# OmerMersin/video-stab

Measured on AMD Instinct MI355X. Metric: stabilized frames/sec @1080p (whole job; warp-stage HBM GB/s in roofline), higher is better.
Workload: dtype u8

## Files before the change

video-stab_amd/csrc/k_lk.hip:

```cpp
#include "vs_common.h"

namespace vsd {
namespace {

constexpr int MAX_LEVELS = 8;

struct LKArgs {
    LKLevel levels[MAX_LEVELS];
    int max_level;
    const float* prev_pts;
    float* next_pts;
    uint8_t* status;
    float* err;
    int n;
    const int32_t* d_n;
    int win;
    int max_count;
    double eps2;
};

template <int CTRL>
__device__ __forceinline__ int dpp_mov(int v) {
    return __builtin_amdgcn_update_dpp(0, v, CTRL, 0xF, 0xF, true);
}
// ... 29 lines not shown
}

__device__ __forceinline__ int descale(int x, int n) { return (x + (1 << (n - 1))) >> n; }

struct Weights { int w00, w01, w10, w11; };

__device__ __forceinline__ Weights make_weights(float a, float b) {
    Weights w;
    w.w00 = f_round((1.f - a) * (1.f - b) * 16384.f);
    w.w01 = f_round(a * (1.f - b) * 16384.f);
    w.w10 = f_round((1.f - a) * b * 16384.f);
    w.w11 = 16384 - w.w00 - w.w01 - w.w10;
    return w;
}

__device__ __forceinline__ short2 load_deriv(const int16_t* __restrict__ d, int w, int h, int x, int y) {
    if ((unsigned)x >= (unsigned)w || (unsigned)y >= (unsigned)h) return make_short2(0, 0);
    return *reinterpret_cast<const short2*>(d + ((size_t)y * w + x) * 2);
}

typedef const __attribute__((address_space(1))) uint8_t* gmem_u8;
typedef const __attribute__((address_space(1))) int16_t* gmem_i16;
__device__ __forceinline__ gmem_u8 uniform_global(const uint8_t* p) {
    const unsigned long long v = (unsigned long long)p;
    const unsigned lo = (unsigned)__builtin_amdgcn_readfirstlane((int)(unsigned)v), hi = (unsigned)__builtin_amdgcn_readfirstlane((int)(unsigned)(v >> 32));
    return (gmem_u8)(((unsigned long long)hi << 32) | lo);
}

constexpr int LK_MARGIN = 6;
constexpr int LK_WIN_MAX = 31;



__device__ __forceinline__ void divmod_small(int i, int d, float inv_d, int& q, int& r) {
    q = (int)(((float)i + 0.5f) * inv_d);
    r = i - q * d;
}

template <int NPX>
__device__ __forceinline__ void lk_track(const LKArgs& a, const int pt) {
    constexpr int WM = NPX <= 4 ? 16 : (NPX <= 7 ? 21 : LK_WIN_MAX);
    constexpr int PWM = WM + 1, RWM = WM + 1 + 2 * LK_MARGIN;
    constexpr int PN = (PWM * PWM + 63) / 64, RN = (RWM * RWM + 63) / 64;
    __shared__ uint8_t pI[PN * 64];
    __shared__ short2 pD[PN * 64];
    __shared__ uint8_t region[RN * 64];
    const int lane = threadIdx.x;
    int n = a.n;
    if (a.d_n) { int dn = *a.d_n; n = dn < n ? dn : n; }
    if (pt >= n) return;
    const int win = a.win, area = win * win;
    const int PW = win + 1;
    const int RW = win + 1 + 2 * LK_MARGIN;
    const float inv_pw = 1.0f / (float)PW, inv_rw = 1.0f / (float)RW, inv_win = 1.0f / (float)win;
    uint32_t off[NPX];
#pragma unroll
    for (int k = 0; k < NPX; k++) {
        const int p = lane + 64 * k;
        int yy = 0, xx = 0;
        if (p < area) divmod_small(p, win, inv_win, yy, xx);
        off[k] = (uint32_t)(yy * PW + xx) | ((uint32_t)(yy * RW + xx) << 16);
    }
#define LK_VALID(k) (lane + 64 * (k) < area)
#define LK_POFF(k) ((int)(off[k] & 0xFFFFu))
#define LK_ROFF(k) ((int)(off[k] >> 16))
    int p_y0, p_x0, p_sy, p_sx, r_y0, r_x0, r_sy, r_sx;
    divmod_small(lane, PW, inv_pw, p_y0, p_x0);
    divmod_small(64, PW, inv_pw, p_sy, p_sx);
    divmod_small(lane, RW, inv_rw, r_y0, r_x0);
    divmod_small(64, RW, inv_rw, r_sy, r_sx);
    const float halfWin = (win - 1) * 0.5f;
    const float FLT_SCALE = 1.f / (1 << 20);
    const float px0 = a.prev_pts[2 * pt], py0 = a.prev_pts[2 * pt + 1];
    float outx = 0.f, outy = 0.f;
    int status = 1;
    float err = 0.f;

    for (int level = a.max_level; level >= 0; level--) {
        const LKLevel L = a.levels[level];
        const float scale = (float)(1. / (double)(1 << level));
        float prevx = px0 * scale, prevy = py0 * scale;
        if (level == a.max_level) { outx = prevx; outy = prevy; }
        else { outx = outx * 2.f; outy = outy * 2.f; }
        prevx -= halfWin; prevy -= halfWin;
        const int ipx = f_floor(prevx), ipy = f_floor(prevy);
        if (ipx < -win || ipx >= L.w || ipy < -win || ipy >= L.h) {
            if (level == 0) { status = 0; err = 0.f; }
            continue;
        }
        float cx = outx - halfWin, cy = outy - halfWin;
        int rx0 = f_floor(cx) - LK_MARGIN, ry0 = f_floor(cy) - LK_MARGIN;
        __syncthreads();
        const bool p_inside = ipx >= 0 && ipy >= 0 && ipx + PW <= L.w && ipy + PW <= L.h;
        if (p_inside) {
            const gmem_u8 pbase = uniform_global(L.prev + ((size_t)ipy * L.stride + ipx));
            const gmem_i16 dbase = (gmem_i16)uniform_global(reinterpret_cast<const uint8_t*>(L.deriv + ((size_t)ipy * L.w + ipx) * 2));
            constexpr int PB_ = 5;
            int y = p_y0, x = p_x0;
#pragma unroll
            for (int k0 = 0; k0 < PN; k0 += PB_) {
                uint8_t vI[PB_];
                uint32_t vD[PB_];
#pragma unroll
                for (int k = k0; k < k0 + PB_ && k < PN; k++) {
                    const bool ok = lane + 64 * k < PW * PW;
                    const uint32_t eo = ok ? (uint32_t)(y * (int)L.stride + x) : 0u, dof = ok ? (uint32_t)((y * L.w + x) * 2) : 0u;
                    vI[k - k0] = pbase[eo];
                    vD[k - k0] = *reinterpret_cast<const __attribute__((address_space(1))) uint32_t*>(dbase + dof);
                    x += p_sx; y += p_sy;
                    if (x >= PW) { x -= PW; y++; }
                }
#pragma unroll
                for (int k = k0; k < k0 + PB_ && k < PN; k++) { pI[lane + 64 * k] = vI[k - k0]; *reinterpret_cast<uint32_t*>(&pD[lane + 64 * k]) = vD[k - k0]; }
                __builtin_amdgcn_sched_barrier(0);
            }
        } else {
            int y = p_y0, x = p_x0;
            for (int i = lane; i < PW * PW; i += 64) {
                const int X = ipx + x, Y = ipy + y;
                pI[i] = L.prev[(size_t)reflect101(Y, L.h) * L.stride + reflect101(X, L.w)];
                pD[i] = load_deriv(L.deriv, L.w, L.h, X, Y);
                x += p_sx; y += p_sy;
                if (x >= PW) { x -= PW; y++; }
            }
        }
        auto stage_region = [&]() {
            const bool inside = rx0 >= 0 && ry0 >= 0 && rx0 + RW <= L.w && ry0 + RW <= L.h;
            int y = r_y0, x = r_x0;
            asm volatile("" : "+v"(x), "+v"(y));
            if (inside) {
                const gmem_u8 rbase = uniform_global(L.next + ((size_t)ry0 * L.stride + rx0));
                constexpr int RB_ = 10;
#pragma unroll
                for (int k0 = 0; k0 < RN; k0 += RB_) {
                    uint8_t vR[RB_];
#pragma unroll
                    for (int k = k0; k < k0 + RB_ && k < RN; k++) {
                        const bool ok = lane + 64 * k < RW * RW;
// ... 4 lines not shown
#pragma unroll
                    for (int k = k0; k < k0 + RB_ && k < RN; k++) region[lane + 64 * k] = vR[k - k0];
                    __builtin_amdgcn_sched_barrier(0);
                }
            } else {
                for (int i = lane; i < RW * RW; i += 64) {
                    const int X = rx0 + x, Y = ry0 + y;
                    region[i] = L.next[(size_t)reflect101(Y, L.h) * L.stride + reflect101(X, L.w)];
                    x += r_sx; y += r_sy;
                    if (x >= RW) { x -= RW; y++; }
                }
            }
        };
        stage_region();
        __syncthreads();
        Weights wt = make_weights(prevx - ipx, prevy - ipy);
        short Iw[NPX], Ix[NPX], Iy[NPX];
        int pA11 = 0, pA12 = 0, pA22 = 0;
#pragma unroll
        for (int k = 0; k < NPX; k++) {
            const int o = LK_POFF(k);
            int ival = descale(__mul24((int)pI[o], wt.w00) + __mul24((int)pI[o + 1], wt.w01) +
                               __mul24((int)pI[o + PW], wt.w10) + __mul24((int)pI[o + PW + 1], wt.w11), 9);
            const short2 d00 = pD[o], d01 = pD[o + 1], d10 = pD[o + PW], d11 = pD[o + PW + 1];
            int ixval = descale(__mul24((int)d00.x, wt.w00) + __mul24((int)d01.x, wt.w01) +
                                __mul24((int)d10.x, wt.w10) + __mul24((int)d11.x, wt.w11), 14);
            int iyval = descale(__mul24((int)d00.y, wt.w00) + __mul24((int)d01.y, wt.w01) +
                                __mul24((int)d10.y, wt.w10) + __mul24((int)d11.y, wt.w11), 14);
            if (!LK_VALID(k)) { ival = 0; ixval = 0; iyval = 0; }
            Iw[k] = (short)ival; Ix[k] = (short)ixval; Iy[k] = (short)iyval;
            pA11 += __mul24(ixval, ixval);
            pA12 += __mul24(ixval, iyval);
            pA22 += __mul24(iyval, iyval);
        }
        const long long sA11 = wave_sum(pA11), sA12 = wave_sum(pA12), sA22 = wave_sum(pA22);
        const float A11 = (float)sA11 * FLT_SCALE, A12 = (float)sA12 * FLT_SCALE, A22 = (float)sA22 * FLT_SCALE;
        float D = A11 * A22 - A12 * A12;
        const float minEig = (A22 + A11 - sqrtf((A11 - A22) * (A11 - A22) + 4.f * A12 * A12)) /
                             (float)(2 * win * win);
// ... 161 lines not shown
    if (!d_prev || !d_next || w <= 0 || h <= 0 || max_level < 0 || max_level >= MAX_LEVELS) {
        set_last_error("pyr_lk: invalid argument");
        return VS_ERR_INVALID_ARG;
    }
    int lw[MAX_LEVELS], lh[MAX_LEVELS];
    int levels = 0;
    {
        int sw = w, sh = h;
        for (int level = 0; level <= max_level; level++) {
            lw[level] = sw; lh[level] = sh;
            levels = level;
            sw = (sw + 1) / 2; sh = (sh + 1) / 2;
            if (sw <= win || sh <= win) break;
        }
    }
    size_t img_bytes = 0, der_bytes = 0;
    for (int i = 1; i <= levels; i++) img_bytes += (size_t)lw[i] * lh[i];
    for (int i = 0; i <= levels; i++) der_bytes += (size_t)lw[i] * lh[i] * 4;
    uint8_t* scratch = nullptr;
    const size_t total = 2 * img_bytes + der_bytes + 64;
    VS_HIP_TRY(hipMalloc((void**)&scratch, total));
    LKLevel L[MAX_LEVELS];
    uint8_t* pp = scratch;
    uint8_t* pn = scratch + img_bytes;
    int16_t* pd = reinterpret_cast<int16_t*>(scratch + ((2 * img_bytes + 15) & ~(size_t)15));
    int rc = VS_OK;
    for (int i = 0; i <= levels && rc == VS_OK; i++) {
        L[i].w = lw[i]; L[i].h = lh[i];
        if (i == 0) { L[i].prev = d_prev; L[i].next = d_next; L[i].stride = stride; }
        else {
            rc = launch_pyr_down(L[i - 1].prev, L[i - 1].stride, lw[i - 1], lh[i - 1], pp, lw[i], st);
            if (rc == VS_OK) rc = launch_pyr_down(L[i - 1].next, L[i - 1].stride, lw[i - 1], lh[i - 1], pn, lw[i], st);
            L[i].prev = pp; L[i].next = pn; L[i].stride = lw[i];
            pp += (size_t)lw[i] * lh[i]; pn += (size_t)lw[i] * lh[i];
        }
        if (rc == VS_OK) rc = launch_scharr(L[i].prev, L[i].stride, lw[i], lh[i], pd, st);
        L[i].deriv = pd;
        pd += (size_t)lw[i] * lh[i] * 2;
    }
    if (rc == VS_OK) rc = launch_pyr_lk(L, levels, d_prev_pts, n, nullptr, d_next_pts, d_status, d_err, win, max_iters, eps, st);
    hipError_t e = hipStreamSynchronize(st);
    (void)hipFree(scratch);
    if (rc == VS_OK && e != hipSuccess) { set_last_error(hipGetErrorString(e)); rc = VS_ERR_HIP; }
    return rc;
}

}
```

video-stab_amd/csrc/k_pyr.hip:

```cpp
#include "vs_common.h"

namespace vsd {
namespace {

constexpr int NT = 256;
constexpr int RPB = 4;

__global__ __launch_bounds__(NT) void pyr_down_kernel(const uint8_t* __restrict__ src_, size_t sstride,
                                                      int sw, int sh, uint8_t* __restrict__ dst_,
                                                      size_t dstride, int dw, int dh) {
    const uint8_t* __restrict__ src = src_;
    uint8_t* __restrict__ dst = dst_;
    const int x = blockIdx.x * blockDim.x + threadIdx.x;
    if (x >= dw) return;
    int xi[5];
#pragma unroll
    for (int k = 0; k < 5; k++) xi[k] = reflect101(2 * x + k - 2, sw);
    for (int y = blockIdx.y * RPB; y < min((int)(blockIdx.y + 1) * RPB, dh); y++) {
        int col[5];
#pragma unroll
        for (int j = 0; j < 5; j++) {
            const uint8_t* s = src + (size_t)reflect101(2 * y + j - 2, sh) * sstride;
            col[j] = s[xi[2]] * 6 + (s[xi[1]] + s[xi[3]]) * 4 + s[xi[0]] + s[xi[4]];
        }
// ... 17 lines not shown
    const int a_p = (r0[xp] + r2[xp]) * 3 + r1[xp] * 10;
    const int b_m = r2[xm] - r0[xm];
    const int b_c = r2[x] - r0[x];
    const int b_p = r2[xp] - r0[xp];
    short2 o;
    o.x = (short)(a_p - a_m);
    o.y = (short)((b_p + b_m) * 3 + b_c * 10);
    *reinterpret_cast<short2*>(dst + ((size_t)y * w + x) * 2) = o;
    }
}

constexpr int FT_W = 64, FT_H = 16;
constexpr int FT_PITCH = 72;
constexpr int FT_ROWS = FT_H + 4;

template <bool DOWN>
__global__ __launch_bounds__(NT) void pyr_level_kernel(const ImgPair* __restrict__ sch, const ImgPair* __restrict__ pyr, size_t sstride,
                                                       int w, int h, size_t dstride, int dw, int dh) {
    __shared__ __attribute__((aligned(16))) uint8_t tile[FT_ROWS * FT_PITCH];
    const uint8_t* __restrict__ src = static_cast<const uint8_t*>(sch[blockIdx.z].src);
    int16_t* __restrict__ der = static_cast<int16_t*>(sch[blockIdx.z].dst);
    const int tid = threadIdx.x;
    const int x0 = blockIdx.x * FT_W, y0 = blockIdx.y * FT_H;
    const bool inside = x0 >= 4 && y0 >= 2 && x0 + FT_W + 4 <= w && y0 + FT_H + 2 <= h && (sstride & 3) == 0 && ((uintptr_t)src & 3) == 0;
    if (inside) {
        constexpr int ND = (FT_ROWS * (FT_PITCH / 4) + NT - 1) / NT;
        uint32_t v[ND];
#pragma unroll
        for (int k = 0; k < ND; k++) {
            const int i = min(tid + NT * k, FT_ROWS * (FT_PITCH / 4) - 1);
            const int r = i / (FT_PITCH / 4), c4 = i - r * (FT_PITCH / 4);
            v[k] = *reinterpret_cast<const uint32_t*>(src + (size_t)(y0 - 2 + r) * sstride + (x0 - 4) + 4 * c4);
        }
#pragma unroll
        for (int k = 0; k < ND; k++)
            if (tid + NT * k < FT_ROWS * (FT_PITCH / 4)) reinterpret_cast<uint32_t*>(tile)[tid + NT * k] = v[k];
// ... 1 lines not shown
        constexpr int NB = (FT_ROWS + 2) / 3;
        const int c = tid % FT_PITCH, r0 = tid / FT_PITCH;
        const uint8_t* col = src + reflect101(x0 - 4 + c, w);
        size_t off[NB];
#pragma unroll
        for (int k = 0; k < NB; k++) off[k] = (size_t)reflect101(y0 - 2 + min(r0 + 3 * k, FT_ROWS - 1), h) * sstride;
        uint8_t v[NB];
#pragma unroll
        for (int k = 0; k < NB; k++) v[k] = col[off[k]];
#pragma unroll
        for (int k = 0; k < NB; k++)
            if (r0 + 3 * k < FT_ROWS) tile[(r0 + 3 * k) * FT_PITCH + c] = v[k];
    }
    __syncthreads();
    const uint32_t* T = reinterpret_cast<const uint32_t*>(tile);
    {
        const int r = tid >> 4, c = (tid & 15) * 4;
        const int y = y0 + r, x = x0 + c;
        if (y < h && x < w) {
            int t[3][6];
#pragma unroll
            for (int j = 0; j < 3; j++) {
                const uint32_t* q = T + (r + 1 + j) * (FT_PITCH / 4) + (c >> 2);
                const uint32_t lo = q[0], mid = q[1], hi = q[2];
                t[j][0] = lo >> 24;
                t[j][1] = mid & 255u; t[j][2] = (mid >> 8) & 255u; t[j][3] = (mid >> 16) & 255u; t[j][4] = mid >> 24;
                t[j][5] = hi & 255u;
            }
            int a[6], b[6];
#pragma unroll
            for (int k = 0; k < 6; k++) {
// ... 25 lines not shown
            for (int j = 0; j < 5; j++) {
                const uint32_t lo = q[j * (FT_PITCH / 4)], hi = q[j * (FT_PITCH / 4) + 1];
                const uint32_t four = __builtin_amdgcn_alignbyte(hi, lo, sh);
                const uint32_t fifth = (hi >> (8 * sh)) & 255u;
                col[j] = (int)__builtin_amdgcn_udot4(four, 0x04060401u, fifth, false);
            }
            dst[(size_t)yo * dstride + xo] = (uint8_t)((col[2] * 6 + (col[1] + col[3]) * 4 + col[0] + col[4] + 128) >> 8);
        }
    }
}

}

int launch_pyr_level_batch(const ImgPair* d_scharr_pairs, const ImgPair* d_pyr_pairs, int items, size_t sstride, int w, int h,
                           size_t dstride, hipStream_t st) {
    if (!d_scharr_pairs || items < 1 || items > 65535 || w <= 0 || h <= 0 || h > 65535) {
        set_last_error("pyr_level_batch: invalid argument");
        return VS_ERR_INVALID_ARG;
    }
    const int dw = (w + 1) / 2, dh = (h + 1) / 2;
    dim3 grid((w + FT_W - 1) / FT_W, (h + FT_H - 1) / FT_H, items);
    if (d_pyr_pairs) hipLaunchKernelGGL(pyr_level_kernel<true>, grid, dim3(NT), 0, st, d_scharr_pairs, d_pyr_pairs, sstride, w, h, dstride, dw, dh);
    else hipLaunchKernelGGL(pyr_level_kernel<false>, grid, dim3(NT), 0, st, d_scharr_pairs, d_pyr_pairs, sstride, w, h, dstride, dw, dh);
    VS_HIP_TRY(hipGetLastError());
    return VS_OK;
}

int launch_pyr_down(const uint8_t* d_src, size_t sstride, int sw, int sh, uint8_t* d_dst,
                    size_t dstride, hipStream_t st) {
    if (!d_src || !d_dst || sw <= 0 || sh <= 0 || sh > 131070) {
        set_last_error("pyr_down: invalid argument");
        return VS_ERR_INVALID_ARG;
    }
    const int dw = (sw + 1) / 2, dh = (sh + 1) / 2;
    dim3 grid((dw + NT - 1) / NT, (dh + RPB - 1) / RPB);
    hipLaunchKernelGGL(pyr_down_kernel, grid, dim3(NT), 0, st, d_src, sstride, sw, sh, d_dst, dstride, dw, dh);
    VS_HIP_TRY(hipGetLastError());
    return VS_OK;
// ... 15 lines not shown
```

video-stab_amd/csrc/stabilizer.cpp:

```cpp
#include <algorithm>
#include <array>
#include <atomic>
#include <cstring>
#include <cstdlib>
#include <deque>
#include <map>
#include <memory>
#include <mutex>
#include <new>
#include <vector>

#include "canvas.h"
#include "host_helper.h"
#include "traj_state.h"
#include "vs_common.h"
#include "warp_tab.h"

namespace vsd {

struct RansacTables;
int get_ransac_tables(int max_m, int iters, const RansacTables** out);
int launch_ransac(const float* d_from, const float* d_to, const uint8_t* d_status, int n, const int32_t* d_n,
                  float* d_vp, float* d_vc, int32_t* d_m, int min_points, double thr, int iters,
                  const RansacTables* tab, int32_t* d_counts, double* d_model, uint8_t* d_inliers,
// ... 32 lines not shown
int launch_fade_update(uint8_t* d_hist, const uint8_t* d_stab, size_t sstride, int row_bytes, int rows, hipStream_t st);
int launch_make_border(const uint8_t* src, size_t sstride, int w, int h, int cn, uint8_t* dst, size_t dstride,
                       int b, int border, hipStream_t st);
int launch_resize_linear(const uint8_t* d_src, size_t sstride, int sw, int sh, int cn, uint8_t* d_dst,
                         size_t dstride, int dw, int dh, hipStream_t st);

constexpr int FRAME_RING = 128;
constexpr int FRAME_RING_MAX = 192;
constexpr int MAX_PYR = 8;
constexpr int NPYR = 3;
constexpr int BATCH_MAX = 64;
constexpr int EVR = 4;

struct Pyramid {
    uint8_t* img[MAX_PYR] = {};
    int16_t* der[MAX_PYR] = {};
};

}

using namespace vsd;

struct vs_batch;
int group_drain(vs_batch* g);
int group_run(vs_batch* g);
bool group_holds_warps(const vs_batch* g);
vs_batch* group_new_own(vs_stab* s);
void group_delete(vs_batch* g);

struct vs_stab {
    vs_params_c p;
// ... 263 lines not shown
    s->items.assign(B, vs_stab::ItemBufs());
    s->bq.clear(); s->kp_cur = 0; s->kp_next = 1;
    if (s->batch_active && !s->group) {
        s->own = group_new_own(s);
        if (!s->own) return fail(s, VS_ERR_HIP, get_last_error());
        s->group = s->own;
    }
    s->free_slots.clear();
    s->ring_frames = (s->batch_active && B > 32) ? FRAME_RING_MAX : FRAME_RING;
    for (int i = 0; i < s->ring_frames; i++) { s->free_slots.push_back(i); s->slot_valid[i] = false; }
    s->ncap = std::max(s->p.max_corners, 1);
    const int ncap = s->ncap;
    size_t off = 0;
    auto take = [&](size_t bytes) { size_t o = off; off += (bytes + 255) & ~(size_t)255; return o; };
    size_t o_first = take((size_t)480 * 270);
    std::vector<std::array<size_t, MAX_PYR>> o_img(s->npyr), o_der(s->npyr);
    for (int k = 0; k < s->npyr; k++)
        for (int l = 0; l <= s->levels; l++) {
            o_img[k][l] = take((size_t)s->lw[l] * s->lh[l]);
            o_der[k][l] = take((size_t)s->lw[l] * s->lh[l] * 4);
        }
    std::vector<size_t> o_pts(nkp), o_npts(nkp);
    for (int k = 0; k < nkp; k++) { o_pts[k] = take((size_t)ncap * 8); o_npts[k] = take(16); }
    struct ItemOff { size_t next, err, vp, vc, status, inl, m, info, counts, model; };
    std::vector<ItemOff> o_it(B);
    for (int k = 0; k < B; k++) {
        o_it[k].next = take((size_t)ncap * 8); o_it[k].err = take((size_t)ncap * 4);
        o_it[k].vp = take((size_t)ncap * 8); o_it[k].vc = take((size_t)ncap * 8);
        o_it[k].status = take(ncap); o_it[k].inl = take(ncap);
        o_it[k].m = take(16); o_it[k].info = take(16); o_it[k].counts = take((size_t)s->p.ransac_max_iters * 4);
        o_it[k].model = take(48);
    }
    size_t o_traj = take(sizeof(TrajState)), o_M = take(96), o_Minv = take(96), o_dbg = take(sizeof(vs_debug_frame));
    size_t o_MinvB[2] = {take((size_t)BATCH_MAX * 96), take((size_t)BATCH_MAX * 96)};
    int tow, toh;
    out_size(s, w, h, &tow, &toh);
    const size_t o_tabs = take(warp_tabs_ints(std::max(w, tow), std::max(h, toh), WARP_BATCH_MAX) * sizeof(int32_t));
    S_HIP(s, hipMalloc((void**)&s->d_all, off));
    S_HIP(s, hipMemsetAsync(s->d_all, 0, off, s->st));
    uint8_t* b = s->d_all;
    s->d_first_gray = b + o_first;
    for (int k = 0; k < s->npyr; k++)
        for (int l = 0; l <= s->levels; l++) {
            s->pyr[k].img[l] = b + o_img[k][l];
            s->pyr[k].der[l] = (int16_t*)(b + o_der[k][l]);
        }
    for (int k = 0; k < nkp; k++) { s->d_pts[k] = (float*)(b + o_pts[k]); s->d_npts[k] = (int32_t*)(b + o_npts[k]); }
    for (int k = 0; k < B; k++) {
        vs_stab::ItemBufs& it = s->items[k];
        it.next = (float*)(b + o_it[k].next); it.err = (float*)(b + o_it[k].err);
        it.vp = (float*)(b + o_it[k].vp); it.vc = (float*)(b + o_it[k].vc);
        it.status = b + o_it[k].status; it.inliers = b + o_it[k].inl;
        it.m = (int32_t*)(b + o_it[k].m); it.info = (int32_t*)(b + o_it[k].info); it.counts = (int32_t*)(b + o_it[k].counts);
        it.model = (double*)(b + o_it[k].model);
    }
    s->d_next = s->items[0].next; s->d_err = s->items[0].err; s->d_vp = s->items[0].vp; s->d_vc = s->items[0].vc;
    s->d_status = s->items[0].status; s->d_inliers = s->items[0].inliers;
    s->d_m = s->items[0].m; s->d_info = s->items[0].info; s->d_counts = s->items[0].counts; s->d_model = s->items[0].model;
    s->d_traj = (TrajState*)(b + o_traj);
    s->d_M = (float*)(b + o_M); s->d_Minv = (double*)(b + o_Minv); s->d_dbg = (vs_debug_frame*)(b + o_dbg);
    s->d_MinvB[0] = (double*)(b + o_MinvB[0]); s->d_MinvB[1] = (double*)(b + o_MinvB[1]);
// ... 48 lines not shown
    t.gauss_ksize = ks;
    float sum = 0.0f;
    int center = ks / 2;
    for (int i = 0; i < ks; i++) {
        float x = (float)(i - center);
        t.gauss_kernel[i] = std::exp(-(x * x) / (2 * sigma * sigma));
        sum += t.gauss_kernel[i];
    }
    for (int i = 0; i < ks; i++) t.gauss_kernel[i] /= sum;
}

int build_pyramid(vs_stab* s, int k, hipStream_t st) {
    Pyramid& P = s->pyr[k];
    for (int l = 1; l <= s->levels; l++)
        S_TRY(s, launch_pyr_down(P.img[l - 1], s->lw[l - 1], s->lw[l - 1], s->lh[l - 1], P.img[l], s->lw[l], st));
    for (int l = 0; l <= s->levels; l++)
        S_TRY(s, launch_scharr(P.img[l], s->lw[l], s->lw[l], s->lh[l], P.der[l], st));
    return VS_OK;
}

inline size_t src_uv(const vs_stab* s) { return (s->zero_copy && s->in_uv_off) ? s->in_uv_off : (size_t)s->h * s->src_pitch; }
inline size_t dst_uv(const vs_stab* s, const uint8_t* d_out, size_t out_stride) {
    return (d_out != s->d_out && s->out_uv_off) ? s->out_uv_off : (size_t)s->h * out_stride;
}

int enqueue_copy_in(vs_stab* s, int slot, const void* src, size_t stride, hipMemcpyKind kind) {
    if (s->slot_valid[slot]) S_HIP(s, hipStreamWaitEvent(s->st_pre, s->ev_slot[slot], 0));
    StageScope t(s, VS_STAGE_COPY_IN, s->st_pre);
    uint8_t* dst = s->d_ring + (size_t)slot * s->frame_bytes;
    if (s->fmt == VS_FMT_NV12 && kind == hipMemcpyDeviceToDevice && s->in_uv_off) {
        S_HIP(s, hipMemcpy2DAsync(dst, s->row_bytes, src, stride, s->row_bytes, s->h, kind, s->st_pre));
        S_HIP(s, hipMemcpy2DAsync(dst + (size_t)s->h * s->row_bytes, s->row_bytes, (const uint8_t*)src + s->in_uv_off, stride,
// ... 45 lines not shown
        s->pts_cap[q] = mc;
        next_pp = q;
        s->last_detected = true;
        s->last_detect_pp = q;
        s->dbg_det_pts = s->d_pts[q]; s->dbg_det_n = s->d_npts[q];
        s->counters.detections++;
    }

    S_HIP(s, hipStreamWaitEvent(s->st, s->ev_pre[c], 0));
    if (s->pts_pending[pp]) {
        S_HIP(s, hipStreamWaitEvent(s->st, s->pts_event[pp], 0));
        s->pts_pending[pp] = false;
    }
    LKLevel L[MAX_PYR];
    for (int l = 0; l <= s->levels; l++) {
        L[l].prev = s->pyr[pv].img[l]; L[l].next = s->pyr[c].img[l]; L[l].deriv = s->pyr[pv].der[l];
        L[l].w = s->lw[l]; L[l].h = s->lh[l]; L[l].stride = s->lw[l];
    }
    const int cap = s->pts_cap[pp];
    {
        StageScope t(s, VS_STAGE_LK, s->st);
        S_TRY(s, launch_pyr_lk(L, s->levels, s->d_pts[pp], cap, s->d_npts[pp], s->d_next, s->d_status, s->d_err,
                               p.lk_win_size, p.lk_max_iters, p.lk_epsilon, s->st));
    }
    s->last_lk_pp = pp;
    if (s->dbg_delay_us > 0) S_TRY(s, launch_spin(s->dbg_delay_us, s->st));
    {
        StageScope t(s, VS_STAGE_RANSAC, s->st);
        S_TRY(s, launch_ransac(s->d_pts[pp], s->d_next, s->d_status, std::max(cap, 0), s->d_npts[pp], s->d_vp, s->d_vc,
                               s->d_m, 4, p.ransac_threshold, p.ransac_max_iters, s->tab, s->d_counts, s->d_model,
                               s->d_inliers, s->d_info, s->d_traj, &s->tp, s->d_dbg, s->have_prev_gray ? 1 : 0, s->st));
// ... 836 lines not shown
    const vs_params_c &p = a->p, &q = b->p;
    return a->w == b->w && a->h == b->h && a->fmt == b->fmt && a->src_pitch == b->src_pitch && a->zero_copy == b->zero_copy &&
           a->in_uv_off == b->in_uv_off && a->out_uv_off == b->out_uv_off && a->aw == b->aw && a->ah == b->ah && a->levels == b->levels &&
           p.lk_win_size == q.lk_win_size && p.ransac_max_iters == q.ransac_max_iters && p.border_size == q.border_size &&
           p.crop_n_zoom == q.crop_n_zoom && (p.border_size <= 0 || p.border_type == q.border_type);
}

int group_allocate(vs_batch* g) {
    const vs_stab* s0 = g->ref;
    const int cap = g->cap, ngf = g->S * (g->B / 2 + 1);
    size_t off = 0;
    auto take = [&](size_t bytes) { size_t o = off; off += (bytes + 255) & ~(size_t)255; return o; };
    const size_t o_gf = take(gftt_item_bytes() * ngf);
    size_t ho = 0;
    auto htake = [&](size_t bytes) { size_t o = ho; ho += (bytes + 255) & ~(size_t)255; return o; };
    g->ho_pairs = htake(sizeof(ImgPair) * cap * (2 + 2 * MAX_PYR));
    g->ho_lk = htake(lk_item_bytes() * cap); g->ho_rs = htake(ransac_item_bytes() * cap);
    g->ho_tail = htake(tail_item_bytes() * cap); g->ho_seg = htake(tail_seg_bytes() * g->S);
    g->up_bytes = ho;
    g->ho_gf = htake(gftt_item_bytes() * ngf);
    g->h_set_bytes = ho;
    const size_t o_set[2] = {take(g->up_bytes), take(g->up_bytes)};
    const size_t o_ti[2] = {take(tail_in_bytes() * cap), take(tail_in_bytes() * cap)};
    const size_t o_minv[2] = {take((size_t)cap * 96), take((size_t)cap * 96)};
    int tow, toh;
    out_size(s0, s0->w, s0->h, &tow, &toh);
    g->tab_ints = s0->fmt == VS_FMT_NV12 ? nv12_tab_ints(s0->w, s0->h) : (int)warp_tabs_ints(std::max(s0->w, tow), std::max(s0->h, toh), 1);
    size_t o_tabs[2];
    for (auto& o : o_tabs) o = take((size_t)g->tab_ints * cap * sizeof(int32_t));
    G_HIP(g, hipMalloc((void**)&g->d_all, off));
    G_HIP(g, hipMemsetAsync(g->d_all, 0, off, g->st));
// ... 133 lines not shown
        for (const vs_stab::BFrame& b : s->bq) ndue += b.out_due ? 1 : 0;
        if (s->p.smoothing_method == VS_SMOOTH_KALMAN) all_apart = 0;
    }
    const vs_params_c& p0 = s0->p;
    const bool pad = p0.border_size > 0 && !p0.crop_n_zoom;
    const bool crop = p0.border_size > 0 && p0.crop_n_zoom && s0->w - 2 * p0.border_size > 0 && s0->h - 2 * p0.border_size > 0;
    for (vs_stab* s : act) {
        const vs_params_c& p = s->p;
        const int ns = (int)s->bq.size(), first = idx;
        int npad = 0;
        for (int i = 0; i < ns; i++, idx++) {
            const vs_stab::BFrame& b = s->bq[i];
            const vs_stab::ItemBufs& it = s->items[i];
            LKLevel L[MAX_PYR];
            for (int l = 0; l <= s->levels; l++) {
                L[l].prev = s->pyr[b.pv].img[l]; L[l].next = s->pyr[b.c].img[l]; L[l].deriv = s->pyr[b.pv].der[l];
                L[l].w = s->lw[l]; L[l].h = s->lh[l]; L[l].stride = s->lw[l];
            }
            const int cap = std::max(b.lk_cap, 0);
            n_max = std::max(n_max, cap);
            G_TRY(g, lk_fill_item(h_lk + lk_item_bytes() * idx, L, s->levels, s->d_pts[b.lk_buf], cap, s->d_npts[b.lk_buf], it.next, it.status, it.err,
                                  p.lk_win_size, p.lk_max_iters, p.lk_epsilon));
            G_TRY(g, ransac_fill_item(h_rs + ransac_item_bytes() * idx, s->d_pts[b.lk_buf], it.next, it.status, cap, s->d_npts[b.lk_buf], it.vp, it.vc,
                                      it.m, 4, p.ransac_threshold, p.ransac_max_iters, s->tab, it.counts, it.model, it.inliers, it.info, s->d_traj,
                                      &s->tp, s->d_dbg, b.have_prev_gray));
            ransac_item_set_last(h_rs + ransac_item_bytes() * idx, i == ns - 1 ? 1 : 0);
            ransac_item_set_tail_in(h_rs + ransac_item_bytes() * idx, g->d_tin[dset] + tail_in_bytes() * idx);
            double* minv = nullptr;
            WarpTabJob jobs[2] = {{nullptr, nullptr, nullptr, 0, 0}, {nullptr, nullptr, nullptr, 0, 0}};
            if (b.out_due) {
                if (npend > 0 && pend_stride != b.out_stride) return gfail(g, VS_ERR_INVALID_ARG, "batch mode: one output pitch per step");
// ... 22 lines not shown
            G_TRY(g, build_pyramid(s, s->bq[0].pv, g->st_pre));
        }
    }
    {
        const int L = s0->levels;
        int aligned = 1, n_detect = 0;
        for (vs_stab* s : act) for (const vs_stab::BFrame& b : s->bq) n_detect += b.detect ? 1 : 0;
        int n_first = 0, n_rest = 0, i = 0;
        for (vs_stab* s : act)
            for (const vs_stab::BFrame& b : s->bq) {
                const Pyramid& P = s->pyr[b.c];
                const int slot = b.detect ? n_first++ : n_detect + n_rest++;
                h_pairs[slot] = ImgPair{b.frame, P.img[0]};
                if ((uintptr_t)b.frame % 8) aligned = 0;
                for (int l = 1; l <= L; l++) h_pairs[(size_t)l * n + i] = ImgPair{P.img[l - 1], P.img[l]};
                for (int l = 0; l <= L; l++) h_pairs[(size_t)(L + 1 + l) * n + i] = ImgPair{P.img[l], P.der[l]};
                i++;
            }
        ImgPair* const d_pairs = g->d_pairs[dset];
        if (k >= 2) G_HIP(g, hipStreamWaitEvent(g->st_up, g->ev_blk[(k - 2) % 4], 0));
        G_HIP(g, hipMemcpyAsync(g->d_pairs[dset], hset, g->up_bytes, hipMemcpyHostToDevice, g->st_up));
        G_HIP(g, hipEventRecord(g->ev_up[dset], g->st_up));
        G_HIP(g, hipStreamWaitEvent(g->st_pre, g->ev_up[dset], 0));
        {
            StageScope t(g->ref, VS_STAGE_GRAY, g->st_pre);
            const int gfmt = s0->fmt == VS_FMT_NV12 ? VS_FMT_GRAY8 : s0->fmt;
            const int n_a = (n_detect > 0 && n_detect < n) ? n_detect : n;
            G_TRY(g, launch_resize_gray_batch(d_pairs, n_a, s0->src_pitch, s0->w, s0->h, gfmt, s0->aw, s0->aw, s0->ah, aligned, g->st_pre));
            G_HIP(g, hipEventRecord(g->ev_bgray, g->st_pre));
            if (n_a < n)
                G_TRY(g, launch_resize_gray_batch(d_pairs + n_a, n - n_a, s0->src_pitch, s0->w, s0->h, gfmt, s0->aw, s0->aw, s0->ah, aligned, g->st_pre));
        }
        StageScope t(g->ref, VS_STAGE_PYRAMID, g->st_pre);
        for (int l = 0; l <= L; l++)
            G_TRY(g, launch_pyr_level_batch(d_pairs + (size_t)(L + 1 + l) * n, l < L ? d_pairs + (size_t)(l + 1) * n : nullptr, n, s0->lw[l], s0->lw[l],
                                            s0->lh[l], l < L ? s0->lw[l + 1] : 0, g->st_pre));
    }
    if (!g->ready.valid) G_HIP(g, hipEventRecord(g->ev_bpre, g->st_pre));
    int ndet = 0;
    for (vs_stab* s : act) {
        int local = 0;
        for (const vs_stab::BFrame& b : s->bq) {
            if (!b.detect) continue;
            G_TRY(g, gftt_fill_item(h_gf + gftt_item_bytes() * ndet, s->pyr[b.c].img[0], s->aw, s->aw, s->ah, s->pts_cap[b.det_buf], 0.02, 15.0, 3,
                                    s->gws[local], s->d_pts[b.det_buf], s->d_npts[b.det_buf]));
            s->dbg_det_pts = s->d_pts[b.det_buf]; s->dbg_det_n = s->d_npts[b.det_buf];
            s->dbg_gftt_counters = s->gws[local].counters;
            local++; ndet++;
        }
        s->last_detected = s->bq.back().detect;
    }
// ... 210 lines not shown
```

video-stab_amd/csrc/vs_common.h:

```cpp
#ifndef VS_COMMON_H
#define VS_COMMON_H

#include <hip/hip_runtime.h>
#include <cstdlib>
#include <stdint.h>
#include <cfloat>
#include <cmath>
#include <string>

#include "../../include/vs_stab.h"

namespace vsd {

void set_last_error(const std::string& msg);
const char* get_last_error();

#define VS_HIP_TRY(expr)                                                                   \
    do {                                                                                   \
        hipError_t _e = (expr);                                                            \
        if (_e != hipSuccess) {                                                            \
            vsd::set_last_error(std::string(#expr) + ": " + hipGetErrorString(_e));        \
            return (_e == hipErrorNoDevice || _e == hipErrorInvalidDevice ||               \
                    _e == hipErrorInsufficientDriver || _e == hipErrorNoBinaryForGpu)      \
                       ? VS_ERR_NO_DEVICE                                                  \
// ... 80 lines not shown
int launch_resize_gray(const uint8_t* d_src, size_t sstride, int sw, int sh, int fmt,
                       uint8_t* d_dst, size_t dstride, int dw, int dh, hipStream_t st);
struct ImgPair { const void* src; void* dst; };
int launch_resize_gray_batch(const ImgPair* d_pairs, int items, size_t sstride, int sw, int sh, int fmt, size_t dstride,
                             int dw, int dh, int aligned, hipStream_t st);
int launch_pyr_level_batch(const ImgPair* d_scharr_pairs, const ImgPair* d_pyr_pairs, int items, size_t sstride, int w, int h,
                           size_t dstride, hipStream_t st);
int launch_pyr_down(const uint8_t* d_src, size_t sstride, int sw, int sh, uint8_t* d_dst,
                    size_t dstride, hipStream_t st);
int launch_scharr(const uint8_t* d_src, size_t sstride, int w, int h, int16_t* d_dst,
                  hipStream_t st);

struct LKLevel {
    const uint8_t* prev;
    const uint8_t* next;
    const int16_t* deriv;
    int w, h;
    size_t stride;
};
int launch_pyr_lk(const LKLevel* levels, int max_level, const float* d_prev_pts, int n,
                  const int32_t* d_n, float* d_next_pts, uint8_t* d_status, float* d_err, int win,
                  int max_iters, double eps, hipStream_t st);

struct GfttWork {
    float* eig;
    uint64_t* cand;
    int32_t* counters;
    int cap;
};
size_t gftt_work_bytes(int w, int h, int cap);
void gftt_work_carve(void* base, int w, int h, int cap, GfttWork* out);
// ... 7 lines not shown
```

Baseline: 120,600.

## Compute Scharr derivatives inside LK patch instead of precomputed full-frame maps

Drops the per-level full-image Scharr derivative pass and its buffers. The LK kernel now stages a padded intensity patch with a one-pixel border and computes Scharr derivatives on the fly into shared memory, with masking for out-of-bounds pixels. This removes full-frame derivative writes and reads (4 bytes per pixel per level) in the pyramid stage. In exchange each tracked point recomputes derivatives for its window and adds an extra sync. The pyramid launch gains a downsample-only variant.

```diff
diff --git a/video-stab_amd/csrc/k_lk.hip b/video-stab_amd/csrc/k_lk.hip
--- a/video-stab_amd/csrc/k_lk.hip
+++ b/video-stab_amd/csrc/k_lk.hip
@@ -67,13 +67,7 @@
     return w;
 }
 
-__device__ __forceinline__ short2 load_deriv(const int16_t* __restrict__ d, int w, int h, int x, int y) {
-    if ((unsigned)x >= (unsigned)w || (unsigned)y >= (unsigned)h) return make_short2(0, 0);
-    return *reinterpret_cast<const short2*>(d + ((size_t)y * w + x) * 2);
-}
-
 typedef const __attribute__((address_space(1))) uint8_t* gmem_u8;
-typedef const __attribute__((address_space(1))) int16_t* gmem_i16;
 __device__ __forceinline__ gmem_u8 uniform_global(const uint8_t* p) {
     const unsigned long long v = (unsigned long long)p;
     const unsigned lo = (unsigned)__builtin_amdgcn_readfirstlane((int)(unsigned)v), hi = (unsigned)__builtin_amdgcn_readfirstlane((int)(unsigned)(v >> 32));
@@ -94,32 +88,38 @@
 __device__ __forceinline__ void lk_track(const LKArgs& a, const int pt) {
     constexpr int WM = NPX <= 4 ? 16 : (NPX <= 7 ? 21 : LK_WIN_MAX);
     constexpr int PWM = WM + 1, RWM = WM + 1 + 2 * LK_MARGIN;
-    constexpr int PN = (PWM * PWM + 63) / 64, RN = (RWM * RWM + 63) / 64;
-    __shared__ uint8_t pI[PN * 64];
-    __shared__ short2 pD[PN * 64];
+    constexpr int DR = NPX <= 7 ? 3 : 5;
+    constexpr int PPM = (PWM + 2 + 3) & ~3;
+    constexpr int SRM = (PWM + 1 + 3) / 4, NGM = (PWM + DR - 1) / DR;
+    static_assert(SRM * NGM <= 64, "one derivative round per level");
+    constexpr int PN = (PPM * (PWM + 2) + 63) / 64, RN = (RWM * RWM + 63) / 64;
+    constexpr int PBYTES = (PN * 64 > PPM * (NGM * DR + 2) + 4 ? PN * 64 : PPM * (NGM * DR + 2) + 4);
+    __shared__ __attribute__((aligned(16))) uint8_t pI_[4 + PBYTES];
+    uint8_t* const pI = pI_ + 4;
+    __shared__ __attribute__((aligned(16))) short2 pD[(PWM + 1) * PPM];
     __shared__ uint8_t region[RN * 64];
     const int lane = threadIdx.x;
     int n = a.n;
     if (a.d_n) { int dn = *a.d_n; n = dn < n ? dn : n; }
     if (pt >= n) return;
     const int win = a.win, area = win * win;
-    const int PW = win + 1;
+    const int PW = win + 1, PP = (PW + 2 + 3) & ~3;
     const int RW = win + 1 + 2 * LK_MARGIN;
-    const float inv_pw = 1.0f / (float)PW, inv_rw = 1.0f / (float)RW, inv_win = 1.0f / (float)win;
+    const float inv_pp = 1.0f / (float)PP, inv_rw = 1.0f / (float)RW, inv_win = 1.0f / (float)win;
     uint32_t off[NPX];
 #pragma unroll
     for (int k = 0; k < NPX; k++) {
         const int p = lane + 64 * k;
         int yy = 0, xx = 0;
         if (p < area) divmod_small(p, win, inv_win, yy, xx);
-        off[k] = (uint32_t)(yy * PW + xx) | ((uint32_t)(yy * RW + xx) << 16);
+        off[k] = (uint32_t)((yy + 1) * PP + xx + 1) | ((uint32_t)(yy * RW + xx) << 16);
     }
 #define LK_VALID(k) (lane + 64 * (k) < area)
 #define LK_POFF(k) ((int)(off[k] & 0xFFFFu))
 #define LK_ROFF(k) ((int)(off[k] >> 16))
     int p_y0, p_x0, p_sy, p_sx, r_y0, r_x0, r_sy, r_sx;
-    divmod_small(lane, PW, inv_pw, p_y0, p_x0);
-    divmod_small(64, PW, inv_pw, p_sy, p_sx);
+    divmod_small(lane, PP, inv_pp, p_y0, p_x0);
+    divmod_small(64, PP, inv_pp, p_sy, p_sx);
     divmod_small(lane, RW, inv_rw, r_y0, r_x0);
     divmod_small(64, RW, inv_rw, r_sy, r_sx);
     const float halfWin = (win - 1) * 0.5f;
@@ -144,37 +144,32 @@
         float cx = outx - halfWin, cy = outy - halfWin;
         int rx0 = f_floor(cx) - LK_MARGIN, ry0 = f_floor(cy) - LK_MARGIN;
         __syncthreads();
-        const bool p_inside = ipx >= 0 && ipy >= 0 && ipx + PW <= L.w && ipy + PW <= L.h;
-        if (p_inside) {
-            const gmem_u8 pbase = uniform_global(L.prev + ((size_t)ipy * L.stride + ipx));
-            const gmem_i16 dbase = (gmem_i16)uniform_global(reinterpret_cast<const uint8_t*>(L.deriv + ((size_t)ipy * L.w + ipx) * 2));
-            constexpr int PB_ = 5;
+        const int pcount = PP * (PW + 2);
+        if (ipx >= 1 && ipy >= 1 && ipx - 1 + PP <= L.w && ipy + PW + 1 <= L.h) {
+            const gmem_u8 pbase = uniform_global(L.prev + ((size_t)(ipy - 1) * L.stride + (ipx - 1)));
+            constexpr int PB_ = 10;
             int y = p_y0, x = p_x0;
 #pragma unroll
             for (int k0 = 0; k0 < PN; k0 += PB_) {
                 uint8_t vI[PB_];
-                uint32_t vD[PB_];
 #pragma unroll
                 for (int k = k0; k < k0 + PB_ && k < PN; k++) {
-                    const bool ok = lane + 64 * k < PW * PW;
-                    const uint32_t eo = ok ? (uint32_t)(y * (int)L.stride + x) : 0u, dof = ok ? (uint32_t)((y * L.w + x) * 2) : 0u;
-                    vI[k - k0] = pbase[eo];
-                    vD[k - k0] = *reinterpret_cast<const __attribute__((address_space(1))) uint32_t*>(dbase + dof);
+                    const bool ok = lane + 64 * k < pcount;
+                    vI[k - k0] = pbase[ok ? (uint32_t)(y * (int)L.stride + x) : 0u];
                     x += p_sx; y += p_sy;
-                    if (x >= PW) { x -= PW; y++; }
-                }
-#pragma unroll
-                for (int k = k0; k < k0 + PB_ && k < PN; k++) { pI[lane + 64 * k] = vI[k - k0]; *reinterpret_cast<uint32_t*>(&pD[lane + 64 * k]) = vD[k - k0]; }
+                    if (x >= PP) { x -= PP; y++; }
+                }
+#pragma unroll
+                for (int k = k0; k < k0 + PB_ && k < PN; k++) pI[lane + 64 * k] = vI[k - k0];
                 __builtin_amdgcn_sched_barrier(0);
             }
         } else {
             int y = p_y0, x = p_x0;
-            for (int i = lane; i < PW * PW; i += 64) {
-                const int X = ipx + x, Y = ipy + y;
+            for (int i = lane; i < pcount; i += 64) {
+                const int X = ipx - 1 + x, Y = ipy - 1 + y;
                 pI[i] = L.prev[(size_t)reflect101(Y, L.h) * L.stride + reflect101(X, L.w)];
-                pD[i] = load_deriv(L.deriv, L.w, L.h, X, Y);
                 x += p_sx; y += p_sy;
-                if (x >= PW) { x -= PW; y++; }
+                if (x >= PP) { x -= PP; y++; }
             }
         }
         auto stage_region = [&]() {
@@ -209,6 +204,50 @@
         };
         stage_region();
         __syncthreads();
+        {
+            const int sr = (PW + 1 + 3) >> 2;
+            int g, c;
+            divmod_small(lane, sr, 1.0f / (float)sr, g, c);
+            const int y = 1 + g * DR, x = 4 * c;
+            if (y <= PW) {
+                const bool masked = !(ipx >= 0 && ipy >= 0 && ipx + PW <= L.w && ipy + PW <= L.h);
+                int t[3][6];
+                auto load_row = [&](int j, int* tj) {
+                    const uint32_t* q = reinterpret_cast<const uint32_t*>(pI + j * PP) + c;
+                    const uint32_t lo = q[-1], mid = q[0], hi = q[1];
+                    tj[0] = lo >> 24;
+                    tj[1] = mid & 255u; tj[2] = (mid >> 8) & 255u; tj[3] = (mid >> 16) & 255u; tj[4] = mid >> 24;
+                    tj[5] = hi & 255u;
+                };
+                load_row(y - 1, t[0]);
+                load_row(y, t[1]);
+#pragma unroll
+                for (int r = 0; r < DR; r++) {
+                    const int* t0 = t[r % 3];
+                    const int* t1 = t[(r + 1) % 3];
+                    int* t2 = t[(r + 2) % 3];
+                    load_row(y + r + 1, t2);
+                    int av[6], bv[6];
+#pragma unroll
+                    for (int k = 0; k < 6; k++) {
+                        av[k] = (t0[k] + t2[k]) * 3 + t1[k] * 10;
+                        bv[k] = t2[k] - t0[k];
+                    }
+                    uint32_t o[4];
+#pragma unroll
+                    for (int k = 0; k < 4; k++) {
+                        const int dx = av[k + 2] - av[k], dy = (bv[k + 2] + bv[k]) * 3 + bv[k + 1] * 10;
+                        o[k] = ((uint32_t)dx & 0xFFFFu) | ((uint32_t)dy << 16);
+                        if (masked && ((unsigned)(ipx - 1 + x + k) >= (unsigned)L.w || (unsigned)(ipy - 1 + y + r) >= (unsigned)L.h)) o[k] = 0u;
+                    }
+                    if (y + r <= PW) *reinterpret_cast<uint4*>(&pD[(y + r) * PP + x]) = make_uint4(o[0], o[1], o[2], o[3]);
+                    __builtin_amdgcn_sched_barrier(0);
+                }
+            }
+        }
+        __syncthreads();
+#pragma unroll
+        for (int k = 0; k < NPX; k++) asm volatile("" : "+v"(off[k]));
         Weights wt = make_weights(prevx - ipx, prevy - ipy);
         short Iw[NPX], Ix[NPX], Iy[NPX];
         int pA11 = 0, pA12 = 0, pA22 = 0;
@@ -216,8 +255,8 @@
         for (int k = 0; k < NPX; k++) {
             const int o = LK_POFF(k);
             int ival = descale(__mul24((int)pI[o], wt.w00) + __mul24((int)pI[o + 1], wt.w01) +
-                               __mul24((int)pI[o + PW], wt.w10) + __mul24((int)pI[o + PW + 1], wt.w11), 9);
-            const short2 d00 = pD[o], d01 = pD[o + 1], d10 = pD[o + PW], d11 = pD[o + PW + 1];
+                               __mul24((int)pI[o + PP], wt.w10) + __mul24((int)pI[o + PP + 1], wt.w11), 9);
+            const short2 d00 = pD[o], d01 = pD[o + 1], d10 = pD[o + PP], d11 = pD[o + PP + 1];
             int ixval = descale(__mul24((int)d00.x, wt.w00) + __mul24((int)d01.x, wt.w01) +
                                 __mul24((int)d10.x, wt.w10) + __mul24((int)d11.x, wt.w11), 14);
             int iyval = descale(__mul24((int)d00.y, wt.w00) + __mul24((int)d01.y, wt.w01) +
@@ -409,16 +448,13 @@
             if (sw <= win || sh <= win) break;
         }
     }
-    size_t img_bytes = 0, der_bytes = 0;
+    size_t img_bytes = 0;
     for (int i = 1; i <= levels; i++) img_bytes += (size_t)lw[i] * lh[i];
-    for (int i = 0; i <= levels; i++) der_bytes += (size_t)lw[i] * lh[i] * 4;
     uint8_t* scratch = nullptr;
-    const size_t total = 2 * img_bytes + der_bytes + 64;
-    VS_HIP_TRY(hipMalloc((void**)&scratch, total));
+    VS_HIP_TRY(hipMalloc((void**)&scratch, 2 * img_bytes + 64));
     LKLevel L[MAX_LEVELS];
     uint8_t* pp = scratch;
     uint8_t* pn = scratch + img_bytes;
-    int16_t* pd = reinterpret_cast<int16_t*>(scratch + ((2 * img_bytes + 15) & ~(size_t)15));
     int rc = VS_OK;
     for (int i = 0; i <= levels && rc == VS_OK; i++) {
         L[i].w = lw[i]; L[i].h = lh[i];
@@ -429,9 +465,6 @@
             L[i].prev = pp; L[i].next = pn; L[i].stride = lw[i];
             pp += (size_t)lw[i] * lh[i]; pn += (size_t)lw[i] * lh[i];
         }
-        if (rc == VS_OK) rc = launch_scharr(L[i].prev, L[i].stride, lw[i], lh[i], pd, st);
-        L[i].deriv = pd;
-        pd += (size_t)lw[i] * lh[i] * 2;
     }
     if (rc == VS_OK) rc = launch_pyr_lk(L, levels, d_prev_pts, n, nullptr, d_next_pts, d_status, d_err, win, max_iters, eps, st);
     hipError_t e = hipStreamSynchronize(st);
diff --git a/video-stab_amd/csrc/k_pyr.hip b/video-stab_amd/csrc/k_pyr.hip
--- a/video-stab_amd/csrc/k_pyr.hip
+++ b/video-stab_amd/csrc/k_pyr.hip
@@ -55,12 +55,12 @@
 constexpr int FT_PITCH = 72;
 constexpr int FT_ROWS = FT_H + 4;
 
-template <bool DOWN>
+template <bool DER, bool DOWN>
 __global__ __launch_bounds__(NT) void pyr_level_kernel(const ImgPair* __restrict__ sch, const ImgPair* __restrict__ pyr, size_t sstride,
                                                        int w, int h, size_t dstride, int dw, int dh) {
+    static_assert(DER || DOWN, "a level launch produces something");
     __shared__ __attribute__((aligned(16))) uint8_t tile[FT_ROWS * FT_PITCH];
-    const uint8_t* __restrict__ src = static_cast<const uint8_t*>(sch[blockIdx.z].src);
-    int16_t* __restrict__ der = static_cast<int16_t*>(sch[blockIdx.z].dst);
+    const uint8_t* __restrict__ src = static_cast<const uint8_t*>((DER ? sch : pyr)[blockIdx.z].src);
     const int tid = threadIdx.x;
     const int x0 = blockIdx.x * FT_W, y0 = blockIdx.y * FT_H;
     const bool inside = x0 >= 4 && y0 >= 2 && x0 + FT_W + 4 <= w && y0 + FT_H + 2 <= h && (sstride & 3) == 0 && ((uintptr_t)src & 3) == 0;
@@ -92,7 +92,8 @@
     }
     __syncthreads();
     const uint32_t* T = reinterpret_cast<const uint32_t*>(tile);
-    {
+    if (DER) {
+        int16_t* __restrict__ der = static_cast<int16_t*>(sch[blockIdx.z].dst);
         const int r = tid >> 4, c = (tid & 15) * 4;
         const int y = y0 + r, x = x0 + c;
         if (y < h && x < w) {
@@ -148,14 +149,17 @@
 
 int launch_pyr_level_batch(const ImgPair* d_scharr_pairs, const ImgPair* d_pyr_pairs, int items, size_t sstride, int w, int h,
                            size_t dstride, hipStream_t st) {
-    if (!d_scharr_pairs || items < 1 || items > 65535 || w <= 0 || h <= 0 || h > 65535) {
+    if ((!d_scharr_pairs && !d_pyr_pairs) || items < 1 || items > 65535 || w <= 0 || h <= 0 || h > 65535) {
         set_last_error("pyr_level_batch: invalid argument");
         return VS_ERR_INVALID_ARG;
     }
     const int dw = (w + 1) / 2, dh = (h + 1) / 2;
     dim3 grid((w + FT_W - 1) / FT_W, (h + FT_H - 1) / FT_H, items);
-    if (d_pyr_pairs) hipLaunchKernelGGL(pyr_level_kernel<true>, grid, dim3(NT), 0, st, d_scharr_pairs, d_pyr_pairs, sstride, w, h, dstride, dw, dh);
-    else hipLaunchKernelGGL(pyr_level_kernel<false>, grid, dim3(NT), 0, st, d_scharr_pairs, d_pyr_pairs, sstride, w, h, dstride, dw, dh);
+    if (!d_scharr_pairs)
+        hipLaunchKernelGGL((pyr_level_kernel<false, true>), grid, dim3(NT), 0, st, d_scharr_pairs, d_pyr_pairs, sstride, w, h, dstride, dw, dh);
+    else if (d_pyr_pairs)
+        hipLaunchKernelGGL((pyr_level_kernel<true, true>), grid, dim3(NT), 0, st, d_scharr_pairs, d_pyr_pairs, sstride, w, h, dstride, dw, dh);
+    else hipLaunchKernelGGL((pyr_level_kernel<true, false>), grid, dim3(NT), 0, st, d_scharr_pairs, d_pyr_pairs, sstride, w, h, dstride, dw, dh);
     VS_HIP_TRY(hipGetLastError());
     return VS_OK;
 }
diff --git a/video-stab_amd/csrc/stabilizer.cpp b/video-stab_amd/csrc/stabilizer.cpp
--- a/video-stab_amd/csrc/stabilizer.cpp
+++ b/video-stab_amd/csrc/stabilizer.cpp
@@ -70,7 +70,6 @@
 
 struct Pyramid {
     uint8_t* img[MAX_PYR] = {};
-    int16_t* der[MAX_PYR] = {};
 };
 
 }
@@ -364,12 +363,9 @@
     size_t off = 0;
     auto take = [&](size_t bytes) { size_t o = off; off += (bytes + 255) & ~(size_t)255; return o; };
     size_t o_first = take((size_t)480 * 270);
-    std::vector<std::array<size_t, MAX_PYR>> o_img(s->npyr), o_der(s->npyr);
+    std::vector<std::array<size_t, MAX_PYR>> o_img(s->npyr);
     for (int k = 0; k < s->npyr; k++)
-        for (int l = 0; l <= s->levels; l++) {
-            o_img[k][l] = take((size_t)s->lw[l] * s->lh[l]);
-            o_der[k][l] = take((size_t)s->lw[l] * s->lh[l] * 4);
-        }
+        for (int l = 0; l <= s->levels; l++) o_img[k][l] = take((size_t)s->lw[l] * s->lh[l]);
     std::vector<size_t> o_pts(nkp), o_npts(nkp);
     for (int k = 0; k < nkp; k++) { o_pts[k] = take((size_t)ncap * 8); o_npts[k] = take(16); }
     struct ItemOff { size_t next, err, vp, vc, status, inl, m, info, counts, model; };
@@ -391,10 +387,7 @@
     uint8_t* b = s->d_all;
     s->d_first_gray = b + o_first;
     for (int k = 0; k < s->npyr; k++)
-        for (int l = 0; l <= s->levels; l++) {
-            s->pyr[k].img[l] = b + o_img[k][l];
-            s->pyr[k].der[l] = (int16_t*)(b + o_der[k][l]);
-        }
+        for (int l = 0; l <= s->levels; l++) s->pyr[k].img[l] = b + o_img[k][l];
     for (int k = 0; k < nkp; k++) { s->d_pts[k] = (float*)(b + o_pts[k]); s->d_npts[k] = (int32_t*)(b + o_npts[k]); }
     for (int k = 0; k < B; k++) {
         vs_stab::ItemBufs& it = s->items[k];
@@ -473,8 +466,6 @@
     Pyramid& P = s->pyr[k];
     for (int l = 1; l <= s->levels; l++)
         S_TRY(s, launch_pyr_down(P.img[l - 1], s->lw[l - 1], s->lw[l - 1], s->lh[l - 1], P.img[l], s->lw[l], st));
-    for (int l = 0; l <= s->levels; l++)
-        S_TRY(s, launch_scharr(P.img[l], s->lw[l], s->lw[l], s->lh[l], P.der[l], st));
     return VS_OK;
 }
 
@@ -550,7 +541,7 @@
     }
     LKLevel L[MAX_PYR];
     for (int l = 0; l <= s->levels; l++) {
-        L[l].prev = s->pyr[pv].img[l]; L[l].next = s->pyr[c].img[l]; L[l].deriv = s->pyr[pv].der[l];
+        L[l].prev = s->pyr[pv].img[l]; L[l].next = s->pyr[c].img[l];
         L[l].w = s->lw[l]; L[l].h = s->lh[l]; L[l].stride = s->lw[l];
     }
     const int cap = s->pts_cap[pp];
@@ -1417,7 +1408,7 @@
     const size_t o_gf = take(gftt_item_bytes() * ngf);
     size_t ho = 0;
     auto htake = [&](size_t bytes) { size_t o = ho; ho += (bytes + 255) & ~(size_t)255; return o; };
-    g->ho_pairs = htake(sizeof(ImgPair) * cap * (2 + 2 * MAX_PYR));
+    g->ho_pairs = htake(sizeof(ImgPair) * cap * MAX_PYR);
     g->ho_lk = htake(lk_item_bytes() * cap); g->ho_rs = htake(ransac_item_bytes() * cap);
     g->ho_tail = htake(tail_item_bytes() * cap); g->ho_seg = htake(tail_seg_bytes() * g->S);
     g->up_bytes = ho;
@@ -1581,7 +1572,7 @@
             const vs_stab::ItemBufs& it = s->items[i];
             LKLevel L[MAX_PYR];
             for (int l = 0; l <= s->levels; l++) {
-                L[l].prev = s->pyr[b.pv].img[l]; L[l].next = s->pyr[b.c].img[l]; L[l].deriv = s->pyr[b.pv].der[l];
+                L[l].prev = s->pyr[b.pv].img[l]; L[l].next = s->pyr[b.c].img[l];
                 L[l].w = s->lw[l]; L[l].h = s->lh[l]; L[l].stride = s->lw[l];
             }
             const int cap = std::max(b.lk_cap, 0);
@@ -1634,7 +1625,6 @@
                 h_pairs[slot] = ImgPair{b.frame, P.img[0]};
                 if ((uintptr_t)b.frame % 8) aligned = 0;
                 for (int l = 1; l <= L; l++) h_pairs[(size_t)l * n + i] = ImgPair{P.img[l - 1], P.img[l]};
-                for (int l = 0; l <= L; l++) h_pairs[(size_t)(L + 1 + l) * n + i] = ImgPair{P.img[l], P.der[l]};
                 i++;
             }
         ImgPair* const d_pairs = g->d_pairs[dset];
@@ -1652,9 +1642,8 @@
                 G_TRY(g, launch_resize_gray_batch(d_pairs + n_a, n - n_a, s0->src_pitch, s0->w, s0->h, gfmt, s0->aw, s0->aw, s0->ah, aligned, g->st_pre));
         }
         StageScope t(g->ref, VS_STAGE_PYRAMID, g->st_pre);
-        for (int l = 0; l <= L; l++)
-            G_TRY(g, launch_pyr_level_batch(d_pairs + (size_t)(L + 1 + l) * n, l < L ? d_pairs + (size_t)(l + 1) * n : nullptr, n, s0->lw[l], s0->lw[l],
-                                            s0->lh[l], l < L ? s0->lw[l + 1] : 0, g->st_pre));
+        for (int l = 0; l < L; l++)
+            G_TRY(g, launch_pyr_level_batch(nullptr, d_pairs + (size_t)(l + 1) * n, n, s0->lw[l], s0->lw[l], s0->lh[l], s0->lw[l + 1], g->st_pre));
     }
     if (!g->ready.valid) G_HIP(g, hipEventRecord(g->ev_bpre, g->st_pre));
     int ndet = 0;
diff --git a/video-stab_amd/csrc/vs_common.h b/video-stab_amd/csrc/vs_common.h
--- a/video-stab_amd/csrc/vs_common.h
+++ b/video-stab_amd/csrc/vs_common.h
@@ -118,7 +118,6 @@
 struct LKLevel {
     const uint8_t* prev;
     const uint8_t* next;
-    const int16_t* deriv;
     int w, h;
     size_t stride;
 };
```

Measured after the change: 126,600 (median of 6 runs). 1.05x the previous value.
